# luisdamiano/sparseRGPs

Hardware: AMD Instinct MI355X
Metric: sparse-GP objective+gradient evals/sec at n=1e6, m=1024, d=8 (higher is better)
Workload: dtype f64; 1 GPU; C3: Titsias VI ELBO + gradient, n=1000000, m=1024, d=8, ard, P=10, knots fixed; n=1000000, m=1024, d=8, kernel=ard, parallelism=single

## Files before the change

### sparsergps_amd/_build.py

```python
from __future__ import annotations

import os
import shutil
import subprocess

HERE = os.path.dirname(os.path.abspath(__file__))
ROOT = os.path.dirname(HERE)
CSRC = os.path.join(HERE, "csrc")
LIBDIR = os.path.join(HERE, "lib")
LIB = os.path.join(LIBDIR, "libsgp.so")
VARIANT_ROOT = os.path.join(ROOT, "tools", "ab")
SOURCES = ["capi.hip", "k_cov.hip", "k_mfma.hip", "k_dense.hip", "k_lap.hip", "multi.hip"]
CSRC_HEADERS = ["sgp_internal.h", "sgp_probe.h", "sgp_multi.h", "sgp_pool.h", "sgp_syrk_plan.h"]
HEADERS = [*CSRC_HEADERS,
           os.path.join("..", "..", "include", "sgp.h"),
           os.path.join("..", "..", "include", "sgp_diag.h")]
ARCH = "gfx950"


class HipccMissing(RuntimeError):
    """No hipcc on this machine (the only case in which an existing library may be reused)."""


def hipcc():
    for cand in (shutil.which("hipcc"), "/opt/rocm/bin/hipcc"):
        if cand and os.path.exists(cand):
            return cand
    raise HipccMissing("hipcc not found: cannot build libsgp.so")


FILE_FLAGS = {"k_dense.hip": ["-mllvm", "-amdgpu-mfma-vgpr-form"]}


def _compile_flags(src, defs=()):
    return ["-O3", f"--offload-arch={ARCH}", "-std=c++17", "-fPIC", "-Wno-unused-result",
            *FILE_FLAGS.get(src, []), *defs]


def _compile_cmd(cc, src, obj, defs=(), csrc=CSRC):
    return [cc, *_compile_flags(src, defs), "-c", os.path.join(csrc, src), "-o", obj]


LINK_FLAGS = [f"--offload-arch={ARCH}", "-shared", "-fPIC", "-ldl", "-lpthread"]


def _link_cmd(cc, objs, out):
    return [cc, *LINK_FLAGS, "-o", out] + list(objs)


def _stamp(path):
    return path + ".cmd"


def _read_stamp(path):
    try:
        with open(_stamp(path)) as f:
            return f.read()
    except OSError:
        return None


def _write_stamp(path, key):
    with open(_stamp(path), "w") as f:
        f.write(key)


def _obj_key(src, defs):
    return "\0".join([src, *_compile_flags(src, defs)])


def _lib_key(objs):
    return "\0".join([*LINK_FLAGS, *(os.path.basename(o) for o in objs)])


def _obj_stale(obj, key, src, csrc=CSRC):
    if not os.path.exists(obj) or _read_stamp(obj) != key:
        return True
    t = os.path.getmtime(obj)
    deps = [os.path.join(csrc, src)] + [os.path.join(csrc, h) for h in HEADERS]
    return any(os.path.getmtime(p) > t for p in deps if os.path.exists(p))


def _sources(csrc=CSRC):
    return [s for s in SOURCES if csrc == CSRC or os.path.exists(os.path.join(csrc, s))]


def _plan(outdir, defs, csrc=CSRC):
    objs, todo = [], []
    for src in _sources(csrc):
        obj = os.path.join(outdir, src.replace(".hip", ".o"))
        objs.append(obj)
        if _obj_stale(obj, _obj_key(src, defs), src, csrc):
            todo.append((src, obj))
    return objs, todo


def _lib_stale(lib, objs):
    if not os.path.exists(lib) or _read_stamp(lib) != _lib_key(objs):
        return True
    t = os.path.getmtime(lib)
    return any(os.path.getmtime(o) > t for o in objs)


def _build_into(outdir, lib, defs, force, verbose, csrc=CSRC):
    cc = hipcc()
    os.makedirs(outdir, exist_ok=True)
    objs, todo = _plan(outdir, defs, csrc)
    if force:
        todo = list(zip(_sources(csrc), objs))
    procs = []
    for src, obj in todo:
        cmd = _compile_cmd(cc, src, obj, defs, csrc)
        procs.append((src, cmd, obj,
                      subprocess.Popen(cmd, stdout=subprocess.PIPE, stderr=subprocess.STDOUT)))
    failed = None
    for src, cmd, obj, p in procs:
        out, _ = p.communicate()
        if p.returncode != 0:
            failed = failed or f"hipcc failed ({' '.join(cmd)}):\n{out.decode(errors='replace')}"
            continue
        _write_stamp(obj, _obj_key(src, defs))
        if verbose and out:
            print(out.decode(errors="replace"))
    if failed:
        raise RuntimeError(failed)
    if not force and not todo and not _lib_stale(lib, objs):
        return lib
    tmp = lib + ".tmp"
    res = subprocess.run(_link_cmd(cc, objs, tmp), stdout=subprocess.PIPE, stderr=subprocess.STDOUT)
    if res.returncode != 0:
        raise RuntimeError(f"link failed:\n{res.stdout.decode(errors='replace')}")
    os.replace(tmp, lib)
    _write_stamp(lib, _lib_key(objs))
    return lib


def stale() -> bool:
    objs, todo = _plan(LIBDIR, ())
    return bool(todo) or _lib_stale(LIB, objs)


def build(force: bool = False, verbose: bool = False) -> str:
    if os.environ.get("SGP_HIPCC_DEFS"):
        raise RuntimeError("SGP_HIPCC_DEFS is not honoured by the product build; "
                           "use sparsergps_amd._build.build_variant() for A/B libraries")
    return _build_into(LIBDIR, LIB, (), force, verbose)


def build_variant(name: str, defs=(), force: bool = False, verbose: bool = False,
                  rev: str | None = None) -> str:
    if not name or "/" in name or name.startswith("."):
        raise ValueError(f"bad variant name {name!r}")
    defs = ["-DSGP_PROBE_BUILD", *defs]
    outdir = os.path.join(VARIANT_ROOT, name)
    csrc = CSRC
    if rev is not None:
        src_root = os.path.join(outdir, "src")
        os.makedirs(src_root, exist_ok=True)
        for path in ["sparsergps_amd/csrc/" + f for f in SOURCES + CSRC_HEADERS] + ["include/sgp.h", "include/sgp_diag.h"]:
            res = subprocess.run(["git", "-C", ROOT, "show", f"{rev}:{path}"],
                                 stdout=subprocess.PIPE, stderr=subprocess.PIPE)
            if res.returncode != 0:
                continue
            out = res.stdout
            dst = os.path.join(src_root, path)
            os.makedirs(os.path.dirname(dst), exist_ok=True)
            old = open(dst, "rb").read() if os.path.exists(dst) else None
            if old != out:
                with open(dst, "wb") as f:
                    f.write(out)
        csrc = os.path.join(src_root, "sparsergps_amd", "csrc")
    return _build_into(outdir, os.path.join(outdir, "libsgp.so"), defs, force, verbose, csrc)


if __name__ == "__main__":
    import sys
    if len(sys.argv) > 2 and sys.argv[1] == "variant":
        rest = sys.argv[3:]
        rev = rest.pop(0) if rest and not rest[0].startswith("-") else None
        print(build_variant(sys.argv[2], rest, verbose=True, rev=rev))
    else:
        print(build(force=True, verbose=True))
```

### sparsergps_amd/csrc/k_mfma.hip

```cpp
#include <algorithm>
#include <vector>

#include "sgp_internal.h"
#include "sgp_probe.h"
#include "sgp_syrk_plan.h"

namespace {

constexpr int T128 = 128;
constexpr int BK = 16;
constexpr int SB = 144;
constexpr int SA = 17;
constexpr int SYRK_RGRP = 16;

__device__ __forceinline__ double wave_sum(double v) {
#pragma unroll
  for (int o = 32; o > 0; o >>= 1) v += __shfl_xor(v, o, 64);
  return v;
}

__device__ __forceinline__ int64_t xcd_remap(int64_t orig, int64_t nwg) {
  return sgp_plan::xcd_remap(orig, nwg);
}

__device__ __forceinline__ void load8(const double* __restrict__ g, double2 (&v)[4]) {
  const double2* p = reinterpret_cast<const double2*>(g);
#pragma unroll
  for (int q = 0; q < 4; ++q) v[q] = p[q];
}
__device__ __forceinline__ void store8(double* s, const double2 (&v)[4]) {
  double2* p = reinterpret_cast<double2*>(s);
#pragma unroll
  for (int q = 0; q < 4; ++q) p[q] = v[q];
}

__device__ __forceinline__ void syrk_group(int64_t gi, int nb, int wv, int& ta, int& tb, int& rs,
                                           int& cs, int& rp, int& cp) {
  const int64_t noff = (int64_t)nb * (nb - 1) / 2;
  if (gi < noff) {
    int a = (int)((sqrtf(8.0f * (float)gi + 1.0f) + 1.0f) * 0.5f);
    while ((int64_t)a * (a - 1) / 2 > gi) --a;
    while ((int64_t)(a + 1) * a / 2 <= gi) ++a;
    const int b = (int)(gi - (int64_t)a * (a - 1) / 2);
    ta = a; tb = b;
    const int wr = wv >> 1, wc = wv & 1;
    rs = wr; cs = 2 + wc;
    rp = 2 * a + wr; cp = 2 * b + wc;
    return;
  }
  const int g = (int)(gi - noff), G = (3 * nb + 3) / 4;
  const int te = G + g / 3, kind = g % 3;
  ta = g;
  tb = (te < nb) ? te : g;
  if (wv == 0) { rs = 0; cs = 0; rp = 2 * g; cp = 2 * g; }
  else if (wv == 1) { rs = 1; cs = 0; rp = 2 * g + 1; cp = 2 * g; }
  else if (wv == 2) { rs = 1; cs = 1; rp = 2 * g + 1; cp = 2 * g + 1; }
  else if (te < nb) {
    if (kind == 0) { rs = 2; cs = 2; rp = 2 * te; cp = 2 * te; }
    else if (kind == 1) { rs = 3; cs = 2; rp = 2 * te + 1; cp = 2 * te; }
    else { rs = 3; cs = 3; rp = 2 * te + 1; cp = 2 * te + 1; }
  } else {
    rs = cs = rp = cp = -1;
  }
}

struct SyrkTMap {
  signed char e[128];
  int S;
};

template <bool SPREAD = false, int PAT = 0, int NVMEM = 8, int NMFMA = 64>
__device__ __forceinline__ void mfma_interleave() {
#pragma unroll
  for (int i = 0; i < NMFMA; ++i) {
    __builtin_amdgcn_sched_group_barrier(0x008, 1, 0);
    if (i >= SGP_IL_VMEM0 && i < SGP_IL_VMEM0 + NVMEM)
      __builtin_amdgcn_sched_group_barrier(0x020, 1, 0);
    if (SPREAD ? (i & 1) == 0 : i < 32)
      __builtin_amdgcn_sched_group_barrier(0x100, 1, 0);
    constexpr int w0 = PAT == 2 ? NMFMA - 8 : PAT == 3 ? NMFMA / 2 : NMFMA - 16;
    if (PAT != 4 && i >= w0 && i < w0 + 8)
      __builtin_amdgcn_sched_group_barrier(0x200, 1, 0);
  }
}

template <int V, int WMODE, int TMODE, bool COMPACT = false>
__device__ __forceinline__ void syrk_dt_body(const double* __restrict__ K, int64_t mp,
                                             const double* __restrict__ w,
                                             const double* __restrict__ r,
                                             const double* __restrict__ tv, int t, int64_t rbeg,
                                             int nsteps, double (*Ka)[BK * SB], double (*ws)[BK],
                                             double (*rw)[BK], double& tacc, double& rrp,
                                             double* __restrict__ out) {
  constexpr int R0 = V, R1 = 7 - V, N0 = R0 + 1, N1 = R1 + 1;
  constexpr bool WITH_T = TMODE != 0;
  const int tid = threadIdx.x, lane = tid & 63;
  d4 acc0[N0], acc1[N1];
#pragma unroll
  for (int c = 0; c < N0; ++c) acc0[c] = d4{0.0, 0.0, 0.0, 0.0};
#pragma unroll
  for (int c = 0; c < N1; ++c) acc1[c] = d4{0.0, 0.0, 0.0, 0.0};
  const int lrow = tid >> 4, lc = tid & 15;
  const double2* gA = reinterpret_cast<const double2*>(K + (rbeg + lrow) * mp + t * (int64_t)T128) + lc;
  const int64_t gstep = BK * mp / 2;
  double2 v[4];
  double vw = 1.0, vsa = 1.0, vrr = 0.0, vr = 0.0;
  double t4[4] = {0.0, 0.0, 0.0, 0.0};
  const int tcol = tid & (T128 - 1), trow = tid >> 7;
#define SDT_GLOAD(step)                                                         \
  {                                                                             \
    const int64_t o_ = (int64_t)(step) * gstep;                                 \
    const int64_t rr_ = rbeg + (int64_t)(step) * BK + (tid & (BK - 1));        \
    _Pragma("unroll") for (int q = 0; q < 4; ++q) v[q] = gA[o_ + 16 * q];       \
    if constexpr (WMODE == 1) vw = w[rr_];                                      \
    if constexpr (WMODE == 2) vsa = w[rbeg + (int64_t)(step) * BK + lrow];      \
    if constexpr (WITH_T) {                                                     \
      vrr = r[rr_];                                                             \
      if constexpr (TMODE == 2) vr = tv[rr_];                                   \
    }                                                                           \
  }
#define SDT_SSTORE(buf, fold)                                                   \
  {                                                                             \
    double2* p_ = reinterpret_cast<double2*>(&Ka[buf][lrow * SB]) + lc;         \
    _Pragma("unroll") for (int q = 0; q < 4; ++q) {                             \
      double2 x_ = v[q];                                                        \
      if constexpr (WMODE == 2) { x_.x *= vsa; x_.y *= vsa; }                   \
      p_[16 * q] = x_;                                                          \
    }                                                                           \
    if constexpr (WMODE == 1) ws[buf][tid & (BK - 1)] = vw;                     \
    if constexpr (WITH_T) {                                                     \
      const double rw_ = TMODE == 2 ? vr : vw * vrr;                            \
      rw[buf][tid & (BK - 1)] = rw_;                                            \
      rrp = fma(rw_ * (fold), vrr, rrp);                                        \
    }                                                                           \
  }
  if (nsteps > 0) {
    SDT_GLOAD(0);
    SDT_SSTORE(0, 1.0);
  }
  __syncthreads();
  for (int step = 0; step < nsteps; ++step) {
    const int cur = step & 1;
    const bool more = step + 1 < nsteps;
    SDT_GLOAD(more ? step + 1 : step);
    const double* Kc = Ka[cur];
#pragma unroll
    for (int kk = 0; kk < 4; ++kk) {
      const int krow = kk * 4 + (lane >> 4);
      const double* row = Kc + krow * SB + (lane & 15);
      double a0 = row[R0 * 16], a1 = row[R1 * 16];
      if constexpr (WMODE == 1) {
        const double wk = ws[cur][krow];
        a0 *= wk;
        a1 *= wk;
      }
#pragma unroll
      for (int c = 0; c < N1; ++c) {
        const double b = row[c * 16];
        if (c < N0) acc0[c] = __builtin_amdgcn_mfma_f64_16x16x4f64(a0, b, acc0[c], 0, 0, 0);
        acc1[c] = __builtin_amdgcn_mfma_f64_16x16x4f64(a1, b, acc1[c], 0, 0, 0);
      }
    }
    if constexpr (WITH_T) {
#pragma unroll
      for (int k = 0; k < BK / 2; ++k) {
        const int q = trow + 2 * k;
        t4[k & 3] = fma(rw[cur][q], Kc[q * SB + tcol], t4[k & 3]);
      }
    }
    SDT_SSTORE(cur ^ 1, more ? 1.0 : 0.0);
    if constexpr (SGP_SDT_IL && WMODE != 1) mfma_interleave<false, 2, 4, 36>();
    __syncthreads();
  }
#undef SDT_GLOAD
#undef SDT_SSTORE
  tacc = (t4[0] + t4[1]) + (t4[2] + t4[3]);
#pragma unroll
  for (int c = 0; c < N1; ++c)
#pragma unroll
    for (int hh = 0; hh < 2; ++hh) {
      if (hh == 0 && c >= N0) continue;
      const int R = hh == 0 ? R0 : R1;
      const d4& a = hh == 0 ? acc0[c] : acc1[c];
      const int rp = 2 * t + R / 4, cp = 2 * t + c / 4;
      double* blk = out + (COMPACT ? (int64_t)(R / 4 + c / 4)
                                   : (int64_t)(rp * (rp + 1) / 2 + cp)) * 4096;
#pragma unroll
      for (int q = 0; q < 4; ++q)
        blk[((R % 4) * 16 + (lane >> 4) + 4 * q) * 64 + (c % 4) * 16 + (lane & 15)] = a[q];
    }
}

template <int WMODE, int TMODE>
__device__ __forceinline__ void syrk_dtile(const double* __restrict__ K, int64_t n_pad,
                                           int64_t mp, const double* __restrict__ w,
                                           const double* __restrict__ r,
                                           const double* __restrict__ tv, int t, int nb,
                                           int64_t sd, int64_t chunk, double (*Ka)[BK * SB],
                                           double (*ws)[BK], double (*rw)[BK],
                                           double* __restrict__ out,
                                           double* __restrict__ slab_t,
                                           double* __restrict__ slab_rr) {
  const int64_t rbeg = sd * chunk;
  int64_t rend = rbeg + chunk;
  if (rend > n_pad) rend = n_pad;
  const int nsteps = rend > rbeg ? (int)((rend - rbeg) / BK) : 0;
  double tacc = 0.0, rrp = 0.0;
  switch (threadIdx.x >> 6) {
    case 0: syrk_dt_body<0, WMODE, TMODE>(K, mp, w, r, tv, t, rbeg, nsteps, Ka, ws, rw, tacc, rrp, out); break;
    case 1: syrk_dt_body<1, WMODE, TMODE>(K, mp, w, r, tv, t, rbeg, nsteps, Ka, ws, rw, tacc, rrp, out); break;
    case 2: syrk_dt_body<2, WMODE, TMODE>(K, mp, w, r, tv, t, rbeg, nsteps, Ka, ws, rw, tacc, rrp, out); break;
    default: syrk_dt_body<3, WMODE, TMODE>(K, mp, w, r, tv, t, rbeg, nsteps, Ka, ws, rw, tacc, rrp, out); break;
  }
  if constexpr (TMODE != 0) {
    const int tid = threadIdx.x;
    double* tsh = &Ka[0][0];
    tsh[tid] = tacc;
    __syncthreads();
    if (tid < T128) slab_t[(sd * nb + t) * T128 + tid] = tsh[tid] + tsh[tid + T128];
    if (t == 0 && tid < 64) {
      double v = tid < BK ? rrp : 0.0;
#pragma unroll
      for (int o = 32; o > 0; o >>= 1) v += __shfl_xor(v, o, 64);
      if (tid == 0) slab_rr[sd] = v;
    }
  }
}

template <int TMODE, int WMODE, int TR = 2>
__global__ void __launch_bounds__(256, 2)
k_syrk_blk(const double* __restrict__ K, int64_t n_pad, int64_t mp, const double* __restrict__ w,
           const double* __restrict__ r, const double* __restrict__ tv,
           int64_t chunk, int ngroups, int nb, double* __restrict__ slab,
           double* __restrict__ slab_t, double* __restrict__ slab_rr, SyrkTMap tm,
           int64_t nwg_blk, int64_t chunk_d, double* __restrict__ slab_d) {
  __shared__ __attribute__((aligned(16))) double Ka[2][BK * SB];
  __shared__ __attribute__((aligned(16))) double Kb[2][BK * SB];
  __shared__ double ws[2][BK];
  __shared__ double rw[2][BK];

  if constexpr (TMODE == 0 || WMODE == 3) {
    if ((int64_t)blockIdx.x >= nwg_blk) {
      const int64_t loc = (int64_t)blockIdx.x - nwg_blk;
      const int t = (int)(loc % nb);
      const int64_t sd = loc / nb;
      syrk_dtile<WMODE == 3 ? 1 : WMODE, TMODE>(
          K, n_pad, mp, w, r, tv, t, nb, sd, chunk_d, Ka, ws, rw,
          slab_d + sd * ((int64_t)(2 * nb) * (2 * nb + 1) / 2) * 4096, slab_t, slab_rr);
      return;
    }
  }
  const int64_t nwg = nwg_blk;
  const int64_t wgid = xcd_remap(blockIdx.x, nwg);
  const int split = (int)(wgid / ngroups);
  const int64_t gi = wgid % ngroups;
  const int tid = threadIdx.x, lane = tid & 63, wv = tid >> 6;
  int ta, tb, rs, cs, rp, cp;
  syrk_group(gi, nb, wv, ta, tb, rs, cs, rp, cp);
  const bool active = rs >= 0;
  const int64_t noff = (int64_t)nb * (nb - 1) / 2;
  const int dg = (gi >= noff) ? (int)(gi - noff) : -1;
  constexpr bool WITH_T = TMODE != 0 && WMODE != 3;
  constexpr bool with_t = WITH_T;
  static_assert(!(WMODE == 2 && TMODE != 0), "sqrt(w)-scaled images: S only");
  constexpr bool SCALE_A = WMODE == 2 || WMODE == 3, SCALE_B = WMODE == 2;
  int tmap = -1;
  if (with_t) {
    if (tm.S > 0) tmap = (int)tm.e[gi];
    else if (gi < noff) tmap = (tb == 0) ? ta : -1;
    else if (dg == 0) tmap = 0;
  }
  const int tS = (with_t && tm.S > 0) ? tm.S : 1, tW = T128 / tS;
  const int tpan = tmap >= 0 ? tmap / tS : -1;
  const int tng = 256 / tW, trg = tid / tW;
  const int tcol = tmap >= 0 ? (tmap % tS) * tW + tid % tW : 0;
  const bool t_on = with_t && tmap >= 0;
  const bool t_inb = tpan != ta;
  const bool t_rr = with_t && dg == 0 && tid < BK;
  double rrp = 0.0;
  double tacc4[4] = {0.0, 0.0, 0.0, 0.0}, vrr = 0.0, vr = 0.0;
  const int64_t rbeg = (int64_t)split * chunk;
  int64_t rend = rbeg + chunk;
  if (rend > n_pad) rend = n_pad;
  const int nsteps = (int)((rend - rbeg) / BK);

  d4 acc[4][4];
#pragma unroll
  for (int a = 0; a < 4; ++a)
#pragma unroll
    for (int b = 0; b < 4; ++b) acc[a][b] = d4{0.0, 0.0, 0.0, 0.0};

  const int lrow = tid >> 4, lc = tid & 15;
  constexpr bool has_tv = TMODE == 2;
  const double2* gA = reinterpret_cast<const double2*>(K + (rbeg + lrow) * mp + ta * (int64_t)T128) + lc;
  const double2* gB = reinterpret_cast<const double2*>(K + (rbeg + lrow) * mp + tb * (int64_t)T128) + lc;
  const int64_t gstep = BK * mp / 2;
  double2 va0, va1, va2, va3, vb0, vb1, vb2, vb3;
  double vw = 1.0, vsa = 1.0;
  const int ra = (rs >> 1) & 1, ro = (rs & 1) * 64;
  const int ca_ = (cs >> 1) & 1, co = (cs & 1) * 64;

#define SYRKB_GLOAD(step)                                                       \
  {                                                                             \
    const int64_t o_ = (int64_t)(step) * gstep;                                 \
    va0 = gA[o_]; va1 = gA[o_ + 16]; va2 = gA[o_ + 32]; va3 = gA[o_ + 48];      \
    vb0 = gB[o_]; vb1 = gB[o_ + 16]; vb2 = gB[o_ + 32]; vb3 = gB[o_ + 48];      \
              \
    const int64_t rr_ = rbeg + (int64_t)(step) * BK + (tid & (BK - 1));        \
    if constexpr (WMODE == 1) vw = w[rr_];                                      \
    if constexpr (SCALE_A) vsa = w[rbeg + (int64_t)(step) * BK + lrow];        \
    if constexpr (WITH_T) {                                                     \
      vrr = r[rr_];                                                             \
      if constexpr (has_tv) vr = tv[rr_];                                       \
    }                                                                           \
  }
#define SYRKB_SSTORE(buf, fold)                                                 \
  {                                                                             \
    double2* pa_ = reinterpret_cast<double2*>(&Ka[buf][lrow * SB]) + lc;        \
    double2* pb_ = reinterpret_cast<double2*>(&Kb[buf][lrow * SB]) + lc;        \
    if constexpr (SCALE_A) {              \
      va0.x *= vsa; va0.y *= vsa; va1.x *= vsa; va1.y *= vsa;                   \
      va2.x *= vsa; va2.y *= vsa; va3.x *= vsa; va3.y *= vsa;                   \
    }                                                                           \
    if constexpr (SCALE_B) {                                                    \
      vb0.x *= vsa; vb0.y *= vsa; vb1.x *= vsa; vb1.y *= vsa;                   \
      vb2.x *= vsa; vb2.y *= vsa; vb3.x *= vsa; vb3.y *= vsa;                   \
    }                                                                           \
    pa_[0] = va0; pa_[16] = va1; pa_[32] = va2; pa_[48] = va3;                  \
    pb_[0] = vb0; pb_[16] = vb1; pb_[32] = vb2; pb_[48] = vb3;                  \
    if constexpr (WMODE == 1) ws[buf][tid & (BK - 1)] = vw;                     \
    if constexpr (WITH_T) {                                                     \
      double rw_;                                          \
      if constexpr (has_tv) rw_ = vr;                                           \
      else rw_ = vw * vrr;                                                      \
      rw[buf][tid & (BK - 1)] = rw_;                                            \
      rrp = fma(rw_ * (fold), vrr, rrp);       \
// ... 388 lines not shown
  d4 acc0[N0], acc1[N1];
#pragma unroll
  for (int c = 0; c < N0; ++c) acc0[c] = d4{0.0, 0.0, 0.0, 0.0};
#pragma unroll
  for (int c = 0; c < N1; ++c) acc1[c] = d4{0.0, 0.0, 0.0, 0.0};
  const int lrow = tid >> 4, lc = tid & 15;
  const double2* gK = reinterpret_cast<const double2*>(K + (rbeg + lrow) * 256) + lc;
  constexpr int64_t gstep = BK * 256 / 2;
  double2 v[8];
  double vw = 1.0;
#define S256_GLOAD(step)                                                        \
  {                                                                             \
    const int64_t o_ = (int64_t)(step) * gstep;                                 \
    _Pragma("unroll") for (int q = 0; q < 8; ++q) v[q] = gK[o_ + 16 * q];       \
    if constexpr (WEIGHTED) vw = w[rbeg + (int64_t)(step) * BK + (tid & (BK - 1))]; \
  }
#define S256_SSTORE(buf)                                                        \
  {                                                                             \
    double2* p_ = reinterpret_cast<double2*>(&Ks[buf][lrow * SB2]) + lc;        \
    _Pragma("unroll") for (int q = 0; q < 8; ++q) p_[16 * q] = v[q];            \
    if constexpr (WEIGHTED) ws[buf][tid & (BK - 1)] = vw;                       \
  }
  if (nsteps > 0) {
    S256_GLOAD(0);
    S256_SSTORE(0);
  }
  __syncthreads();
  for (int step = 0; step < nsteps; ++step) {
    const int cur = step & 1;
    S256_GLOAD(step + 1 < nsteps ? step + 1 : step);
    const double* Kc = Ks[cur];
#pragma unroll
    for (int kk = 0; kk < 4; ++kk) {
      const int krow = kk * 4 + (lane >> 4);
      const double* row = Kc + krow * SB2 + (lane & 15);
      double a0 = row[R0 * 16], a1 = row[R1 * 16];
      if constexpr (WEIGHTED) {
        const double wk = ws[cur][krow];
        a0 *= wk;
        a1 *= wk;
      }
#pragma unroll
      for (int c = 0; c < N1; ++c) {
        const double b = row[c * 16];
        if (c < N0) acc0[c] = __builtin_amdgcn_mfma_f64_16x16x4f64(a0, b, acc0[c], 0, 0, 0);
        acc1[c] = __builtin_amdgcn_mfma_f64_16x16x4f64(a1, b, acc1[c], 0, 0, 0);
      }
    }
    S256_SSTORE(cur ^ 1);
    if constexpr (SGP_S256_IL) mfma_interleave<false, 2, 8, 68>();
    __syncthreads();
  }
#undef S256_GLOAD
#undef S256_SSTORE
#pragma unroll
  for (int c = 0; c < N1; ++c)
#pragma unroll
    for (int hh = 0; hh < 2; ++hh) {
      if (hh == 0 && c >= N0) continue;
      const int R = hh == 0 ? R0 : R1;
      const d4& a = hh == 0 ? acc0[c] : acc1[c];
      const int rp = R / 4, cp = c / 4;
      double* blk = out + (int64_t)(rp * (rp + 1) / 2 + cp) * 4096;
#pragma unroll
      for (int q = 0; q < 4; ++q)
        blk[((R % 4) * 16 + (lane >> 4) + 4 * q) * 64 + (c % 4) * 16 + (lane & 15)] = a[q];
    }
}

template <bool WEIGHTED>
__global__ void __launch_bounds__(256, 2)
k_syrk_s256(const double* __restrict__ K, int64_t n_pad, const double* __restrict__ w,
            int64_t chunk, double* __restrict__ slab) {
  __shared__ __attribute__((aligned(16))) double Ks[2][BK * SB2];
  __shared__ double ws[2][BK];
  const int64_t nwg = (int64_t)gridDim.x;
  const int64_t wgid = xcd_remap(blockIdx.x, nwg);
  const int64_t split = wgid >> 1;
  const int v = (int)(wgid & 1) * 4 + (threadIdx.x >> 6);
  const int64_t rbeg = split * chunk;
  int64_t rend = rbeg + chunk;
  if (rend > n_pad) rend = n_pad;
  const int nsteps = rend > rbeg ? (int)((rend - rbeg) / BK) : 0;
  double* out = slab + split * 10 * 4096;
#define S256_CASE(v_)                                                          \
  case v_:                                                                     \
    syrk256_body<v_, WEIGHTED>(K, w, rbeg, nsteps, Ks, ws, out);               \
    break;
  switch (v) {
    S256_CASE(0) S256_CASE(1) S256_CASE(2) S256_CASE(3)
    S256_CASE(4) S256_CASE(5) S256_CASE(6) S256_CASE(7)
  }
#undef S256_CASE
}

__global__ void __launch_bounds__(256, 2)
k_gemm_tn(const double* __restrict__ A, int64_t lda, const double* __restrict__ B, int64_t ldb,
          int64_t n_pad, int nta, int ntb, int64_t chunk, double* __restrict__ slab) {
  __shared__ __attribute__((aligned(16))) double Ka[2][BK * SB];
  __shared__ __attribute__((aligned(16))) double Kb[2][BK * SB];
  const int64_t nwg = (int64_t)gridDim.x;
  const int64_t wgid = xcd_remap(blockIdx.x, nwg);
  const int ntile = nta * ntb;
  const int split = (int)(wgid / ntile);
  const int tile = (int)(wgid % ntile);
  const int ta = tile / ntb, tb = tile % ntb;
  const int tid = threadIdx.x, lane = tid & 63, wv = tid >> 6;
  const int wr = wv >> 1, wc = wv & 1;
  const int64_t rbeg = (int64_t)split * chunk;
  int64_t rend = rbeg + chunk;
  if (rend > n_pad) rend = n_pad;
  const int nsteps = (int)((rend - rbeg) / BK);
  d4 acc[4][4];
#pragma unroll
  for (int a = 0; a < 4; ++a)
#pragma unroll
    for (int b = 0; b < 4; ++b) acc[a][b] = d4{0.0, 0.0, 0.0, 0.0};
  const int lrow = tid >> 4, lc = tid & 15;
  const double2* gA = reinterpret_cast<const double2*>(A + (rbeg + lrow) * lda + ta * (int64_t)T128) + lc;
  const double2* gB = reinterpret_cast<const double2*>(B + (rbeg + lrow) * ldb + tb * (int64_t)T128) + lc;
  const int64_t sa = BK * lda / 2, sb = BK * ldb / 2;
  double2 va0, va1, va2, va3, vb0, vb1, vb2, vb3;
#define TN_GLOAD(step)                                                          \
  {                                                                             \
    const int64_t oa_ = (int64_t)(step) * sa, ob_ = (int64_t)(step) * sb;       \
    va0 = gA[oa_]; va1 = gA[oa_ + 16]; va2 = gA[oa_ + 32]; va3 = gA[oa_ + 48];  \
    vb0 = gB[ob_]; vb1 = gB[ob_ + 16]; vb2 = gB[ob_ + 32]; vb3 = gB[ob_ + 48];  \
  }
#define TN_SSTORE(buf)                                                          \
  {                                                                             \
    double2* pa_ = reinterpret_cast<double2*>(&Ka[buf][lrow * SB]) + lc;        \
    double2* pb_ = reinterpret_cast<double2*>(&Kb[buf][lrow * SB]) + lc;        \
    pa_[0] = va0; pa_[16] = va1; pa_[32] = va2; pa_[48] = va3;                  \
    pb_[0] = vb0; pb_[16] = vb1; pb_[32] = vb2; pb_[48] = vb3;                  \
  }
  if (nsteps > 0) {
    TN_GLOAD(0);
    TN_SSTORE(0);
  }
  __syncthreads();
  for (int step = 0; step < nsteps; ++step) {
    const int cur = step & 1;
    if (step + 1 < nsteps) TN_GLOAD(step + 1);
    const double* As = Ka[cur];
    const double* Bs = Kb[cur];
#pragma unroll
    for (int kk = 0; kk < 4; ++kk) {
      const int krow = kk * 4 + (lane >> 4);
      double af[4], bf[4];
#pragma unroll
      for (int f = 0; f < 4; ++f) {
        af[f] = As[krow * SB + wr * 64 + f * 16 + (lane & 15)];
        bf[f] = Bs[krow * SB + wc * 64 + f * 16 + (lane & 15)];
      }
#pragma unroll
      for (int fm = 0; fm < 4; ++fm)
#pragma unroll
        for (int fn = 0; fn < 4; ++fn)
          acc[fm][fn] = __builtin_amdgcn_mfma_f64_16x16x4f64(af[fm], bf[fn], acc[fm][fn], 0, 0, 0);
    }
    if (step + 1 < nsteps) TN_SSTORE(cur ^ 1);
    __syncthreads();
  }
#undef TN_GLOAD
#undef TN_SSTORE
  double* out = slab + ((int64_t)split * ntile + tile) * (T128 * T128);
#pragma unroll
  for (int fm = 0; fm < 4; ++fm)
#pragma unroll
    for (int fn = 0; fn < 4; ++fn)
#pragma unroll
      for (int q = 0; q < 4; ++q) {
        const int row = wr * 64 + fm * 16 + (lane >> 4) + 4 * q;
        const int col = wc * 64 + fn * 16 + (lane & 15);
        out[row * T128 + col] = acc[fm][fn][q];
      }
}

__global__ void __launch_bounds__(256)
k_gemm_tn_reduce(const double* __restrict__ slab, int splits, int nta, int ntb,
                 double* __restrict__ C) {
  const int tile = blockIdx.y;
  const int e = blockIdx.x * 256 + threadIdx.x;
  const int ntile = nta * ntb;
  double s = 0.0;
  for (int sp = 0; sp < splits; ++sp) s += slab[((int64_t)sp * ntile + tile) * (T128 * T128) + e];
  const int ta = tile / ntb, tb = tile % ntb;
  const int64_t a = (int64_t)ta * T128 + e / T128, b = (int64_t)tb * T128 + e % T128;
  C[a * (int64_t)ntb * T128 + b] = s;
}

__global__ void __launch_bounds__(256)
k_syrk_reduce_t(const double* __restrict__ slab_t, const double* __restrict__ slab_rr,
                int splits, int nb, int64_t mp, double* __restrict__ red) {
  const int64_t a = (int64_t)blockIdx.x * 256 + threadIdx.x;
  if (a < mp) {
    const int ta = (int)(a / T128), col = (int)(a % T128);
    double s = 0.0;
    for (int sp = 0; sp < splits; ++sp) s += slab_t[((int64_t)sp * nb + ta) * T128 + col];
    red[mp * mp + a] = s;
  }
  if (blockIdx.x == 0 && threadIdx.x == 0) {
    double s = 0.0;
    for (int sp = 0; sp < splits; ++sp) s += slab_rr[sp];
    red[mp * mp + mp] = s;
  }
}

enum { EPI_GRAD = 0, EPI_ROWQUAD = 1 };

constexpr int CON_A_SZ = T128 * SA;
constexpr int CON_B_SZ = BK * SB;
constexpr int CON_LDS = 2 * (CON_A_SZ + CON_B_SZ);

enum { CON_FULL = 0, CON_TAIL = 1, CON_HEAD = 2 };
constexpr int64_t CON_SK_SLOT = 65 * 256;
struct ConSK {
  double* ws = nullptr;
  int dp = -1;
  unsigned* flags = nullptr;
  unsigned epoch = 0;
  int64_t slot = 0;
  int* status = nullptr;
};

__device__ __forceinline__ unsigned con_ldu_sc1(const unsigned* p) {
  return __hip_atomic_load(p, __ATOMIC_RELAXED, __HIP_MEMORY_SCOPE_AGENT);
}

template <int DT, int EPI, bool V2, bool KNOT, bool FROM_T, bool KU, bool T2, int SKM,
          bool VIF = false>
__device__ __forceinline__ void con_tile(
    const KernParams& kp, const double* __restrict__ K, const double* __restrict__ M,
    const double* __restrict__ X, int64_t ldx, int64_t n, int64_t n_pad,
    const double* __restrict__ U, int64_t ldu, int64_t m, int64_t mp, const ConArgs& ca,
    double* __restrict__ slab, int nrec, double* __restrict__ rowq, int64_t ti, int64_t tj,
    int64_t wgid, int kb, int ke, double* lds, double (*red)[SGP_MAXD + 5], double (*s_uk)[BK],
    const ConSK& sk, int part, int tid_in) {
  const double* __restrict__ r = ca.r;
  const double* __restrict__ uvec = ca.uvec;
  const double* __restrict__ cdiag = ca.cdiag;
  constexpr int A_SZ = CON_A_SZ, B_SZ = CON_B_SZ;
  const int64_t ntj = mp / T128;
  const int64_t nwg = (n_pad / T128) * ntj;
  const int64_t i0 = ti * T128, j0 = tj * T128;

  const int tid = tid_in, lane = tid & 63, wv = tid >> 6;
  const int wr = wv >> 1, wc = wv & 1;
  const bool with_u = KU && (uvec != nullptr) && (ca.alpha_in == nullptr);
  constexpr bool with_v = V2;
  constexpr bool NOCS = VIF && !KNOT;

  d4 acc[4][4];
#pragma unroll
  for (int a = 0; a < 4; ++a)
#pragma unroll
    for (int b = 0; b < 4; ++b) acc[a][b] = d4{0.0, 0.0, 0.0, 0.0};

  const int arow = tid >> 1, acol = (tid & 1) * 8;
  const double2* gA = reinterpret_cast<const double2*>(K + (i0 + arow) * mp + acol);
  const int bk = tid >> 4, bc = tid & 15;
  const double2* gB = reinterpret_cast<const double2*>(M + (int64_t)bk * mp + j0) + bc;
  const int64_t bstep = BK * mp / 2;
  double2 va0, va1, va2, va3, vb0, vb1, vb2, vb3;
  double ku = 0.0, vuk = 0.0;
  const double* __restrict__ uk_src = with_u ? uvec : M;

#define CON_GLOAD(step)                                                          \
  {                                                                              \
    const int64_t oa_ = (int64_t)(step) * (BK / 2), ob_ = (int64_t)(step) * bstep; \
    va0 = gA[oa_]; va1 = gA[oa_ + 1]; va2 = gA[oa_ + 2]; va3 = gA[oa_ + 3];      \
    vb0 = gB[ob_]; vb1 = gB[ob_ + 16]; vb2 = gB[ob_ + 32]; vb3 = gB[ob_ + 48];   \
    if constexpr (KU) vuk = uk_src[(int64_t)(step) * BK + (tid & (BK - 1))];     \
  }
#define CON_SSTORE(buf)                                                          \
  {                                                                              \
    double* As_ = lds + (buf) * (A_SZ + B_SZ);                                   \
    double* pa_ = &As_[arow * SA + acol];                                        \
    double2* pb_ = reinterpret_cast<double2*>(&As_[A_SZ + bk * SB]) + bc;        \
    pa_[0] = va0.x; pa_[1] = va0.y; pa_[2] = va1.x; pa_[3] = va1.y;              \
    pa_[4] = va2.x; pa_[5] = va2.y; pa_[6] = va3.x; pa_[7] = va3.y;              \
    pb_[0] = vb0; pb_[16] = vb1; pb_[32] = vb2; pb_[48] = vb3;                   \
    if constexpr (KU) s_uk[buf][tid & (BK - 1)] = vuk;    \
  }
#define CON_KU(buf)                                                              \
  {                                                                              \
    const double* u_ = &s_uk[buf][acol];                                         \
    ku = fma(va0.x, u_[0], ku); ku = fma(va0.y, u_[1], ku);                      \
    ku = fma(va1.x, u_[2], ku); ku = fma(va1.y, u_[3], ku);                      \
    ku = fma(va2.x, u_[4], ku); ku = fma(va2.y, u_[5], ku);                      \
    ku = fma(va3.x, u_[6], ku); ku = fma(va3.y, u_[7], ku);                      \
  }

  SGP_PROBE_CON_STAMP(0);
  if constexpr (FROM_T) {
#pragma unroll
    for (int fm = 0; fm < 4; ++fm)
#pragma unroll
      for (int fn = 0; fn < 4; ++fn)
#pragma unroll
        for (int q = 0; q < 4; ++q)
          acc[fm][fn][q] = ca.tin[(i0 + wr * 64 + fm * 16 + (lane >> 4) + 4 * q) * mp + j0 +
                                  wc * 64 + fn * 16 + (lane & 15)];
  } else {
  CON_GLOAD(kb);
  CON_SSTORE(0);
  __syncthreads();
  for (int step = kb; step < ke; ++step) {
    const int cur = (step - kb) & 1;
    if constexpr (KU) CON_KU(cur);
    CON_GLOAD(step + 1 < ke ? step + 1 : step);
    const double* As = lds + cur * (A_SZ + B_SZ);
    const double* Bs = As + A_SZ;
#pragma unroll
    for (int kk = 0; kk < 4; ++kk) {
      const int kx = kk * 4 + (lane >> 4);
      double af[4], bf[4];
#pragma unroll
      for (int f = 0; f < 4; ++f) {
        af[f] = As[(wr * 64 + f * 16 + (lane & 15)) * SA + kx];
        bf[f] = Bs[kx * SB + wc * 64 + f * 16 + (lane & 15)];
      }
#pragma unroll
      for (int fm = 0; fm < 4; ++fm)
#pragma unroll
        for (int fn = 0; fn < 4; ++fn)
          acc[fm][fn] = __builtin_amdgcn_mfma_f64_16x16x4f64(af[fm], bf[fn], acc[fm][fn], 0, 0, 0);
    }
    CON_SSTORE(cur ^ 1);
    mfma_interleave<SGP_CON_IL_SPREAD, SGP_CON_IL_PAT>();
    __syncthreads();
  }
  }
#undef CON_GLOAD
#undef CON_SSTORE
#undef CON_KU

  if constexpr (SKM == CON_TAIL) {
    double* w = sk.ws + sk.slot * CON_SK_SLOT;
#pragma unroll
    for (int fm = 0; fm < 4; ++fm)
#pragma unroll
      for (int fn = 0; fn < 4; ++fn)
#pragma unroll
        for (int q = 0; q < 4; ++q)
          __hip_atomic_store(&w[((fm * 4 + fn) * 4 + q) * 256 + tid], acc[fm][fn][q],
                             __ATOMIC_RELAXED, __HIP_MEMORY_SCOPE_AGENT);
    __hip_atomic_store(&w[64 * 256 + tid], ku, __ATOMIC_RELAXED, __HIP_MEMORY_SCOPE_AGENT);
    asm volatile("s_waitcnt vmcnt(0)" ::: "memory");
    __syncthreads();
    if (tid == 0)
      __hip_atomic_store(&sk.flags[sk.slot], sk.epoch, __ATOMIC_RELAXED, __HIP_MEMORY_SCOPE_AGENT);
    return;
  }
  if (SKM == CON_HEAD && part == CON_HEAD) {
    if (tid == 0) {
      unsigned it = 0;
      while (con_ldu_sc1(&sk.flags[sk.slot]) != sk.epoch) {
        if (++it >= (1u << 22)) {
          atomicExch(sk.status, -1);
          break;
        }
        __builtin_amdgcn_s_sleep(1);
      }
    }
    __syncthreads();
    const double* w = sk.ws + sk.slot * CON_SK_SLOT;
#pragma unroll
    for (int fm = 0; fm < 4; ++fm) {
      double t[4][4];
#pragma unroll
      for (int fn = 0; fn < 4; ++fn)
#pragma unroll
        for (int q = 0; q < 4; ++q)
          t[fn][q] = __hip_atomic_load(&w[((fm * 4 + fn) * 4 + q) * 256 + tid], __ATOMIC_RELAXED,
                                       __HIP_MEMORY_SCOPE_AGENT);
#pragma unroll
      for (int fn = 0; fn < 4; ++fn)
#pragma unroll
        for (int q = 0; q < 4; ++q) acc[fm][fn][q] += t[fn][q];
      __builtin_amdgcn_sched_barrier(0);
    }
    ku += __hip_atomic_load(&w[64 * 256 + tid], __ATOMIC_RELAXED, __HIP_MEMORY_SCOPE_AGENT);
  }

  SGP_PROBE_CON_STAMP(1);
  if constexpr (SGP_CON_EPI_PRIO > 0) __builtin_amdgcn_s_setprio(SGP_CON_EPI_PRIO);
  SGP_PROBE_CON_SKIP_EPILOGUE()
  double* s_alpha = lds;
  double* s_rs = s_alpha + T128;
  double* s_u = s_rs + T128;
  double* s_cd = s_u + T128;
  double* s_beta = s_cd + T128;
  double* s_v = s_beta + T128;
  double* s_xs = s_v + T128;
  double* s_us = s_xs + T128 * 16;
  double* s_rs2 = lds + 8320;
  static_assert(8320 + T128 <= 2 * (A_SZ + B_SZ), "s_rs2 fits the LDS image");
  ku += __shfl_xor(ku, 1, 64);
  double a2 = 0.0;
  if ((tid & 1) == 0) {
    const int64_t i = i0 + arow;
    double iz, al;
    if constexpr (VIF) {
      iz = ca.invz;
      al = r[i] * iz;
    } else {
      iz = ca.invz_vec ? ca.invz_vec[i] : ca.invz;
      al = ca.alpha_in ? ca.alpha_in[i]
                       : (with_u ? (r[i] - ku) * iz : 0.0);
    }
    const bool iv = i < n;
    s_alpha[arow] = iv ? al : 0.0;
    s_rs[arow] = iv ? (ca.rs_vec ? ca.rs * ca.rs_vec[i] : ca.rs) : 0.0;
    if constexpr (T2) s_rs2[arow] = iv ? (ca.rs_vec2 ? ca.rs2 * ca.rs_vec2[i] : ca.rs2) : 0.0;
    s_beta[arow] = (with_v && iv) ? ca.beta_in[i] : 0.0;
    if constexpr (!VIF) {
      if (tj == 0) {
        if (ca.count_a2 && i < n) a2 = al * al;
        if (ca.alpha_out) ca.alpha_out[i] = al;
      }
    }
  }
  const double* Kt = K + i0 * mp + j0;

  if constexpr (EPI == EPI_ROWQUAD) {
    if (ca.tstore != nullptr) {
#pragma unroll
      for (int fm = 0; fm < 4; ++fm)
#pragma unroll
        for (int fn = 0; fn < 4; ++fn)
#pragma unroll
          for (int q = 0; q < 4; ++q)
            ca.tstore[(i0 + wr * 64 + fm * 16 + (lane >> 4) + 4 * q) * mp + j0 + wc * 64 +
                      fn * 16 + (lane & 15)] = acc[fm][fn][q];
    }
    __syncthreads();
    double* s_q = s_cd;
#pragma unroll
    for (int fm = 0; fm < 4; ++fm) {
      double kv[4][4];
#pragma unroll
      for (int q = 0; q < 4; ++q)
#pragma unroll
        for (int fn = 0; fn < 4; ++fn)
          kv[q][fn] = Kt[(int64_t)(wr * 64 + fm * 16 + (lane >> 4) + 4 * q) * mp +
                         wc * 64 + fn * 16 + (lane & 15)];
#pragma unroll
      for (int q = 0; q < 4; ++q) {
        const int row = wr * 64 + fm * 16 + (lane >> 4) + 4 * q;
        double v = 0.0;
#pragma unroll
        for (int fn = 0; fn < 4; ++fn)
          v = fma(kv[q][fn], acc[fm][fn][q], v);
        v += __shfl_xor(v, 1, 64);
        v += __shfl_xor(v, 2, 64);
        v += __shfl_xor(v, 4, 64);
        v += __shfl_xor(v, 8, 64);
        if ((lane & 15) == 0) s_q[wc * T128 + row] = v;
      }
    }
    __syncthreads();
    if (tid < T128) rowq[tj * n_pad + i0 + tid] = s_q[tid] + s_q[T128 + tid];
    return;
  } else {
    const int d = kp.d;
    constexpr int sus = 9;
    const bool ard = (kp.kernel == 1);
    const double rl2s = kp.rl2[0];
    const int L = kp.L;
    for (int e = tid; e < T128; e += 256) {
      const int64_t j = j0 + e;
      s_u[e] = (uvec && j < m) ? uvec[j] : 0.0;
      s_v[e] = (with_v && j < m) ? ca.vvec[j] : 0.0;
      s_cd[e] = (cdiag && j < m) ? cdiag[j] : 0.0;
    }
    double e_sig = 0.0;
    double e_sq = 0.0;
    double* s_kn;
    static_assert(DT % 8 == 0, "coordinates are processed in chunks of 8");
    constexpr int NCH = DT / 8;
    {
      constexpr int KST = 136;
      const double* const kq0 = K + (i0 + (wv >> 1) * 64 + 4 * (wv & 1)) * mp + j0 + 2 * lane;
      double* kst = s_us + ((T128 * sus + 1) & ~1);
#define CON_XSTAGE(ch_)                                                                  \
      _Pragma("unroll") for (int e = tid; e < T128 * 8; e += 256) {                      \
        const int rr = e % T128, c = e / T128, cg = 8 * (ch_) + c;                       \
        const int64_t i = i0 + rr, j = j0 + rr;                                          \
        double xv = 0.0;                                                                 \
        if (cg < d) {                                                                    \
          const double sc = ard ? kp.rl[cg] : 1.0;                                       \
          xv = (i < n) ? X[i + cg * ldx] * sc : 0.0;                                     \
          s_us[rr * sus + c] = (j < m) ? U[j + cg * ldu] * sc : 0.0;                     \
        }                                                                                \
        s_xs[rr * 16 + c] = xv;                                                          \
        s_xs[rr * 16 + 8 + c] = xv * xv;                                                 \
      }
#ifdef SGP_CON_PROBE_NO_KDMA
#define CON_KHALF(s_)
#else
#define CON_KHALF(s_)                                                                    \
      _Pragma("unroll") for (int q_ = 0; q_ < 4; ++q_) {                                 \
        const int rho_ = wv * 4 + q_;                                                    \
        __builtin_amdgcn_global_load_lds(                                                \
            (const __attribute__((address_space(1))) void*)(                             \
                kq0 + (int64_t)(((s_) >> 1) * 16 + ((s_) & 1) * 8 + q_) * mp),          \
            (__attribute__((address_space(3))) void*)(kst + ((s_) & 1) * 16 * KST + rho_ * KST), \
            16, 0, 0);                                                                   \
      }
#endif
      double t2n[2][4];
#define CON_T2LOAD(s_)                                                                   \
      if constexpr (T2) {                                                                \
        _Pragma("unroll") for (int r2_ = 0; r2_ < 2; ++r2_)                              \
        _Pragma("unroll") for (int fn_ = 0; fn_ < 4; ++fn_)                              \
          t2n[r2_][fn_] = ca.tin2[(i0 + wr * 64 + ((s_) >> 1) * 16 + (lane >> 4) +        \
                                   4 * (2 * ((s_) & 1) + r2_)) * mp + j0 + wc * 64 +      \
                                  fn_ * 16 + (lane & 15)];                                \
      }
      CON_KHALF(0);
      CON_KHALF(1);
      CON_T2LOAD(0);
      CON_XSTAGE(0);
      __builtin_amdgcn_s_waitcnt(0);
      __syncthreads();
      s_kn = kst;
      SGP_PROBE_CON_STAMP(4);

      d4 P[4];
      double Cc[4], ucol[4], vcol[4];
#pragma unroll
      for (int fn = 0; fn < 4; ++fn) {
        const int col = wc * 64 + fn * 16 + (lane & 15);
        P[fn] = d4{0.0, 0.0, 0.0, 0.0};
        Cc[fn] = 0.0;
        ucol[fn] = s_u[col];
        vcol[fn] = with_v ? s_v[col] : 0.0;
      }
      {
#pragma unroll
        for (int hs = 0; hs < 8; ++hs) {
          const int fm = hs >> 1, h = hs & 1;
          if (hs > 0) {
            __builtin_amdgcn_s_waitcnt(0);
            __syncthreads();
            if (hs < 7) { CON_KHALF(hs + 1); }
          }
          double t2c[2][4];
          if constexpr (T2) {
#pragma unroll
            for (int r2 = 0; r2 < 2; ++r2)
#pragma unroll
              for (int fn = 0; fn < 4; ++fn) t2c[r2][fn] = t2n[r2][fn];
            if (hs < 7) { CON_T2LOAD(hs + 1); }
          }
          const double* kb = kst + h * 16 * KST;
          double xb[2];
#pragma unroll
          for (int r2 = 0; r2 < 2; ++r2)
            xb[r2] = s_xs[(wr * 64 + fm * 16 + 4 * (2 * h + r2) + (lane >> 4)) * 16 + (lane & 15)];
#pragma unroll
          for (int fn = 0; fn < 4; ++fn) {
            const int col = wc * 64 + fn * 16 + (lane & 15);
            double kv[2];
#pragma unroll
            for (int r2 = 0; r2 < 2; ++r2) kv[r2] = kb[(wr * 8 + (lane >> 4) + 4 * r2) * KST + col];
#pragma unroll
            for (int r2 = 0; r2 < 2; ++r2) {
              const int q = 2 * h + r2;
              const int row = wr * 64 + fm * 16 + (lane >> 4) + 4 * q;
              double G = s_rs[row] * acc[fm][fn][q];
              if constexpr (T2) G = fma(s_rs2[row], t2c[r2][fn], G);
              if constexpr (V2) G = fma(s_beta[row], vcol[fn], G);
              G = fma(s_alpha[row], ucol[fn], G);
              double w = G * kv[r2];
              if constexpr ((V2 && KNOT) || FROM_T) w = (j0 + col < m && i0 + row < n) ? w : 0.0;
              if constexpr (!NOCS) Cc[fn] += w;
              acc[fm][fn][q] = w;
            }
          }
#pragma unroll
          for (int r2 = 0; r2 < 2; ++r2)
#pragma unroll
            for (int fn = 0; fn < 4; ++fn)
#ifndef SGP_CON_PROBE_NO_EPI_MFMA
              P[fn] = __builtin_amdgcn_mfma_f64_16x16x4f64(acc[fm][fn][2 * h + r2], xb[r2], P[fn],
                                                           0, 0, 0);
#else
              P[fn][r2] = fma(acc[fm][fn][2 * h + r2], xb[r2], P[fn][r2]);
#endif
          if (hs == 1) SGP_PROBE_CON_STAMP(3);
        }
        __syncthreads();
      }
#undef CON_KHALF
#undef CON_T2LOAD
      SGP_PROBE_CON_STAMP(5);
      const int cp = lane & 15, cc = cp & 7;
#pragma unroll
      for (int ch = 0; ch < NCH; ++ch) {
        if (8 * ch >= d) break;
        if (ch > 0) {
          __syncthreads();
          CON_XSTAGE(ch);
          __syncthreads();
// ... 1035 lines not shown
```

### sparsergps_amd/csrc/sgp_probe.h

```cpp
#pragma once

#if (defined(SGP_CON_TRACE) || defined(SGP_CON_NO_EPILOGUE) || defined(SGP_GJ_TRACE) ||       \
     defined(SGP_IL_VMEM0) || defined(SGP_CON_IL_PAT) || defined(SGP_SYRK_IL_PAT) ||          \
     defined(SGP_CON_IL_SPREAD) || defined(SGP_CON_SHMEM) ||                                  \
     defined(SGP_SYRK_BAL) || defined(SGP_SYRK_WB) || defined(SGP_SYRK_WB_SLOTS) ||           \
     defined(SGP_SDT_IL) || defined(SGP_S256_IL) ||                  \
     defined(SGP_SDT_W) || defined(SGP_SDT_WW) || defined(SGP_SDT_WT) ||                      \
     defined(SGP_SYRK_W3) || defined(SGP_CON_ROWQ_KU) ||                                      \
     defined(SGP_LAP_RS_CFG) || defined(SGP_GJ_MM_UNROLL) || defined(SGP_VI_BUILD_NO_T) ||        \
     defined(SGP_GJ_STEPS) || defined(SGP_GJ_GMAX) || defined(SGP_CHAIN_US_STEP) ||         \
     defined(SGP_CHAIN_US_FIX) || defined(SGP_HOST_PROBE) || defined(SGP_BUILD_OCC_T2) ||      \
     defined(SGP_CON_EPI_PRIO) || defined(SGP_CON_PROBE_NO_EPI_MFMA) ||                       \
     defined(SGP_CON_PROBE_NO_KDMA)) &&      \
    !defined(SGP_PROBE_BUILD)
#error "timing probes and experiment knobs are for variant builds only (SGP_PROBE_BUILD)"
#endif

#ifndef SGP_CON_EPI_PRIO
#define SGP_CON_EPI_PRIO 0
#endif
#ifndef SGP_BUILD_OCC_T2
#define SGP_BUILD_OCC_T2 4
#endif
#ifndef SGP_IL_VMEM0
#define SGP_IL_VMEM0 0
#endif
#ifndef SGP_CON_IL_PAT
#define SGP_CON_IL_PAT 2
#endif
#ifndef SGP_SYRK_IL_PAT
#define SGP_SYRK_IL_PAT 0
#endif
#ifndef SGP_CON_IL_SPREAD
#define SGP_CON_IL_SPREAD false
#endif
#ifndef SGP_CON_SHMEM
#define SGP_CON_SHMEM 0
#endif
#ifndef SGP_SYRK_BAL
#define SGP_SYRK_BAL 1
#endif
#ifndef SGP_SYRK_WB
#define SGP_SYRK_WB 1
#endif
#ifndef SGP_SYRK_WB_SLOTS
#define SGP_SYRK_WB_SLOTS 512
#endif
#ifndef SGP_SDT_IL
#define SGP_SDT_IL 1
#endif
#ifndef SGP_SDT_W
#define SGP_SDT_W 38
#endif
#ifndef SGP_SDT_WW
#define SGP_SDT_WW 2
#endif
#ifndef SGP_SDT_WT
#define SGP_SDT_WT 6
#endif
#ifndef SGP_SYRK_W3
#define SGP_SYRK_W3 1
#endif
#ifndef SGP_CON_ROWQ_KU
#define SGP_CON_ROWQ_KU 0
#endif
#ifndef SGP_LAP_RS_CFG
#define SGP_LAP_RS_CFG 0
#endif
#ifndef SGP_GJ_MM_UNROLL
#define SGP_GJ_MM_UNROLL 16
#endif
#ifndef SGP_S256_IL
#define SGP_S256_IL 0
#endif
#ifndef SGP_GJ_STEPS
#define SGP_GJ_STEPS 0
#endif
#ifndef SGP_GJ_GMAX
#define SGP_GJ_GMAX 128
#endif
#ifndef SGP_CHAIN_US_STEP
#define SGP_CHAIN_US_STEP 60.0
#endif
#ifndef SGP_CHAIN_US_FIX
#define SGP_CHAIN_US_FIX 250.0
#endif
#ifndef SGP_VI_BUILD_NO_T
#define SGP_VI_BUILD_NO_T 0
#endif

#ifdef SGP_CON_TRACE
#define SGP_PROBE_CON_STAMP(k_)        \
  do {                                 \
    if (tid == 0) SGP_CON_TRACE(k_);   \
  } while (0)
#else
#define SGP_PROBE_CON_STAMP(k_) \
  do {                          \
  } while (0)
#endif

#ifdef SGP_CON_NO_EPILOGUE
#define SGP_PROBE_CON_SKIP_EPILOGUE()                                                   \
  if constexpr (EPI == EPI_GRAD) {                                                      \
    double v_ = 0.0;                                                                    \
    _Pragma("unroll") for (int fm_ = 0; fm_ < 4; ++fm_)                                 \
      _Pragma("unroll") for (int fn_ = 0; fn_ < 4; ++fn_)                               \
        v_ += acc[fm_][fn_][0] + acc[fm_][fn_][3];                                      \
    if (v_ == 1234.5) slab[tid] = v_;                                                   \
    return;                                                                             \
  }
#else
#define SGP_PROBE_CON_SKIP_EPILOGUE()
#endif

#ifdef SGP_GJ_TRACE
#define SGP_PROBE_GJ_DECL() const bool gj_tr_ = (i == k + 1) && (j == k + 1) && threadIdx.x == 0
#define SGP_PROBE_GJ_STAMP(p_)          \
  do {                                  \
    if (gj_tr_) SGP_GJ_TRACE(k, p_);    \
  } while (0)
#else
#define SGP_PROBE_GJ_DECL() \
  do {                      \
  } while (0)
#define SGP_PROBE_GJ_STAMP(p_) \
  do {                         \
  } while (0)
#endif
```

Before: 21.40 evals/s.

## Stage contraction k-loop tiles via global_load_lds DMA with swizzled double-buffered LDS

```diff
diff --git a/sparsergps_amd/_build.py b/sparsergps_amd/_build.py
--- a/sparsergps_amd/_build.py
+++ b/sparsergps_amd/_build.py
@@ -11,7 +11,8 @@
 LIB = os.path.join(LIBDIR, "libsgp.so")
 VARIANT_ROOT = os.path.join(ROOT, "tools", "ab")
 SOURCES = ["capi.hip", "k_cov.hip", "k_mfma.hip", "k_dense.hip", "k_lap.hip", "multi.hip"]
-CSRC_HEADERS = ["sgp_internal.h", "sgp_probe.h", "sgp_multi.h", "sgp_pool.h", "sgp_syrk_plan.h"]
+CSRC_HEADERS = ["sgp_internal.h", "sgp_probe.h", "sgp_multi.h", "sgp_pool.h", "sgp_syrk_plan.h",
+                "sgp_kstage.h"]
 HEADERS = [*CSRC_HEADERS,
            os.path.join("..", "..", "include", "sgp.h"),
            os.path.join("..", "..", "include", "sgp_diag.h")]
diff --git a/sparsergps_amd/csrc/k_mfma.hip b/sparsergps_amd/csrc/k_mfma.hip
--- a/sparsergps_amd/csrc/k_mfma.hip
+++ b/sparsergps_amd/csrc/k_mfma.hip
@@ -2,6 +2,7 @@
 #include <vector>
 
 #include "sgp_internal.h"
+#include "sgp_kstage.h"
 #include "sgp_probe.h"
 #include "sgp_syrk_plan.h"
 
@@ -32,6 +33,41 @@
   double2* p = reinterpret_cast<double2*>(s);
 #pragma unroll
   for (int q = 0; q < 4; ++q) p[q] = v[q];
+}
+
+namespace ks = sgp_kstage;
+static_assert(ks::kKStride == SB && ks::kBK == BK && ks::kTile == T128, "sgp_kstage.h's k image");
+
+__device__ __forceinline__ void kst_dma16(const void* gbase, unsigned voff, unsigned lds_dst) {
+  unsigned keep;
+  asm volatile(
+      "s_mov_b32 %0, m0\n\t"
+      "s_mov_b32 m0, %3\n\t"
+      "s_nop 0\n\t"
+      "global_load_lds_dwordx4 %1, %2\n\t"
+      "s_mov_b32 m0, %0"
+      : "=&s"(keep)
+      : "v"(voff), "s"(gbase), "s"(lds_dst)
+      : "memory");
+}
+__device__ __forceinline__ void kst_dma_wait() { asm volatile("s_waitcnt vmcnt(0)" ::: "memory"); }
+__device__ __forceinline__ void kst_step_end() {
+  __builtin_amdgcn_sched_barrier(0);
+  kst_dma_wait();
+  __syncthreads();
+}
+__device__ __forceinline__ unsigned kst_lds_addr(const double* p) {
+  return __builtin_amdgcn_readfirstlane(
+      (unsigned)(uintptr_t)(__attribute__((address_space(3))) const void*)p);
+}
+__device__ __forceinline__ const void* kst_uniform(const void* p) {
+  const uint64_t a = (uint64_t)(uintptr_t)p;
+  const uint32_t lo = __builtin_amdgcn_readfirstlane((uint32_t)a);
+  const uint32_t hi = __builtin_amdgcn_readfirstlane((uint32_t)(a >> 32));
+  return (const void*)(uintptr_t)(((uint64_t)hi << 32) | lo);
+}
+__device__ __forceinline__ double kst_ld(const double* img, int byte_off) {
+  return *reinterpret_cast<const double*>(reinterpret_cast<const char*>(img) + byte_off);
 }
 
 __device__ __forceinline__ void syrk_group(int64_t gi, int nb, int wv, int& ta, int& tb, int& rs,
@@ -1026,6 +1062,67 @@
         for (int q = 0; q < 4; ++q)
           acc[fm][fn][q] = ca.tin[(i0 + wr * 64 + fm * 16 + (lane >> 4) + 4 * q) * mp + j0 +
                                   wc * 64 + fn * 16 + (lane & 15)];
+  } else if constexpr (SGP_KLOOP_DMA && VIF && !KU) {
+    static_assert(ks::kRowImgDoubles <= A_SZ && ks::kKImgDoubles == B_SZ, "DMA images fit the stage");
+    const int wvs = __builtin_amdgcn_readfirstlane(wv);
+    const int64_t rowb = mp * 8;
+    unsigned voa[ks::kInstr];
+#pragma unroll
+    for (int i = 0; i < ks::kInstr; ++i)
+      voa[i] = (unsigned)((ks::row_dma_row(wvs, i, lane) - ks::row_dma_row(wvs, i, 0)) * rowb) +
+               (unsigned)(ks::row_dma_chunk(wvs, i, lane) * ks::kDmaBytes);
+    const unsigned vob = ks::k_dma_chunk(lane) * ks::kDmaBytes;
+    const char* gMs = static_cast<const char*>(kst_uniform(M + j0));
+    const int64_t stepb = BK * rowb;
+    const char* gKr[ks::kInstr];
+    int64_t ko[ks::kInstr];
+#pragma unroll
+    for (int i = 0; i < ks::kInstr; ++i) {
+      gKr[i] = static_cast<const char*>(kst_uniform(K + (i0 + ks::row_dma_row(wvs, i, 0)) * mp));
+      ko[i] = ks::k_dma_krow(wvs, i) * rowb;
+    }
+    const unsigned l0 = kst_lds_addr(lds);
+    constexpr unsigned BUFB = (A_SZ + B_SZ) * 8, BOFF = A_SZ * 8;
+#define CON_DMA2(h, step, buf)                                                              \
+    _Pragma("unroll") for (int q_ = 2 * (h); q_ < 2 * (h) + 2; ++q_) {                      \
+      const int i_ = q_ & 3;                                                                \
+      if (q_ < 4)                                                                           \
+        kst_dma16(gKr[i_] + (int64_t)(step) * (BK * 8),                                     \
+                  voa[i_], l0 + (unsigned)(buf) * BUFB + ks::row_dma_lds(wvs, i_));         \
+      else                                                                                  \
+        kst_dma16(gMs + (int64_t)(step) * stepb + ko[i_], vob,                              \
+                  l0 + (unsigned)(buf) * BUFB + BOFF + ks::k_dma_lds(wvs, i_));             \
+    }
+    CON_DMA2(0, kb, 0);
+    CON_DMA2(1, kb, 0);
+    CON_DMA2(2, kb, 0);
+    CON_DMA2(3, kb, 0);
+    kst_dma_wait();
+    __syncthreads();
+    for (int step = kb; step < ke; ++step) {
+      const int cur = (step - kb) & 1;
+      const int nxt = step + 1 < ke ? step + 1 : step;
+      const double* As = lds + cur * (A_SZ + B_SZ);
+      const double* Bs = As + A_SZ;
+#pragma unroll
+      for (int kk = 0; kk < 4; ++kk) {
+        double af[4], bf[4];
+#pragma unroll
+        for (int f = 0; f < 4; ++f) {
+          af[f] = kst_ld(As, ks::row_frag(wr, f, kk, lane));
+          bf[f] = kst_ld(Bs, ks::k_frag(wc * 64, f, kk, lane));
+        }
+        CON_DMA2(kk, nxt, cur ^ 1);
+#pragma unroll
+        for (int fm = 0; fm < 4; ++fm)
+#pragma unroll
+          for (int fn = 0; fn < 4; ++fn)
+            acc[fm][fn] = __builtin_amdgcn_mfma_f64_16x16x4f64(af[fm], bf[fn], acc[fm][fn], 0, 0, 0);
+      }
+      mfma_interleave<SGP_CON_IL_SPREAD, 4, 0>();
+      kst_step_end();
+    }
+#undef CON_DMA2
   } else {
   CON_GLOAD(kb);
   CON_SSTORE(0);
diff --git a/sparsergps_amd/csrc/sgp_kstage.h b/sparsergps_amd/csrc/sgp_kstage.h
--- /dev/null
+++ b/sparsergps_amd/csrc/sgp_kstage.h
@@ -0,0 +1,65 @@
+#pragma once
+
+#include <stdint.h>
+
+#if defined(__HIPCC__)
+#ifndef SGP_HD
+#define SGP_HD __host__ __device__ inline
+#endif
+#else
+#ifndef SGP_HD
+#define SGP_HD inline
+#endif
+#endif
+
+namespace sgp_kstage {
+
+constexpr int kBK = 16;
+constexpr int kTile = 128;
+constexpr int kWaves = 4;
+constexpr int kLanes = 64;
+constexpr int kInstr = 4;
+constexpr int kDmaBytes = 16;
+constexpr int kPiece = kLanes * kDmaBytes;
+
+constexpr int kRowBytes = kBK * 8;
+constexpr int kRowPad = 128;
+constexpr int kRowImgBytes = kTile * kRowBytes + (kTile / 16) * kRowPad;
+constexpr int kRowImgDoubles = kRowImgBytes / 8;
+
+SGP_HD int row_swz(int row) { return (row >> 1) & 7; }
+SGP_HD int row_base(int row) { return row * kRowBytes + (row >> 4) * kRowPad; }
+
+SGP_HD int row_dma_group(int wave, int i) { return wave * kInstr + i; }
+SGP_HD int row_dma_lds(int wave, int i) { return row_base(row_dma_group(wave, i) * 8); }
+SGP_HD int row_dma_row(int wave, int i, int lane) { return row_dma_group(wave, i) * 8 + (lane >> 3); }
+SGP_HD int row_dma_chunk(int wave, int i, int lane) {
+  return (lane & 7) ^ row_swz(row_dma_row(wave, i, lane));
+}
+SGP_HD int row_elem(int row, int k) {
+  return row_base(row) + (((k >> 1) ^ row_swz(row)) << 4) + ((k & 1) << 3);
+}
+SGP_HD int row_frag_row(int wr, int fm, int lane) { return wr * 64 + fm * 16 + (lane & 15); }
+SGP_HD int row_frag_k(int kk, int lane) { return kk * 4 + (lane >> 4); }
+SGP_HD int row_frag(int wr, int fm, int kk, int lane) {
+  return row_elem(row_frag_row(wr, fm, lane), row_frag_k(kk, lane));
+}
+
+constexpr int kKStride = 144;
+constexpr int kKStrideBytes = kKStride * 8;
+constexpr int kKImgDoubles = kBK * kKStride;
+constexpr int kKImgBytes = kKImgDoubles * 8;
+
+SGP_HD int k_dma_krow(int wave, int i) { return wave * kInstr + i; }
+SGP_HD int k_dma_lds(int wave, int i) { return k_dma_krow(wave, i) * kKStrideBytes; }
+SGP_HD int k_dma_chunk(int lane) { return lane; }
+SGP_HD int k_elem(int k, int col) { return k * kKStrideBytes + col * 8; }
+SGP_HD int k_frag_k(int kk, int lane) { return kk * 4 + (lane >> 4); }
+SGP_HD int k_frag_col(int c0, int f, int lane) { return c0 + f * 16 + (lane & 15); }
+SGP_HD int k_frag(int c0, int f, int kk, int lane) {
+  return k_elem(k_frag_k(kk, lane), k_frag_col(c0, f, lane));
+}
+
+SGP_HD int bank_pair(int byte_off) { return (byte_off >> 3) & 31; }
+
+}
diff --git a/sparsergps_amd/csrc/sgp_probe.h b/sparsergps_amd/csrc/sgp_probe.h
--- a/sparsergps_amd/csrc/sgp_probe.h
+++ b/sparsergps_amd/csrc/sgp_probe.h
@@ -4,7 +4,7 @@
      defined(SGP_IL_VMEM0) || defined(SGP_CON_IL_PAT) || defined(SGP_SYRK_IL_PAT) ||          \
      defined(SGP_CON_IL_SPREAD) || defined(SGP_CON_SHMEM) ||                                  \
      defined(SGP_SYRK_BAL) || defined(SGP_SYRK_WB) || defined(SGP_SYRK_WB_SLOTS) ||           \
-     defined(SGP_SDT_IL) || defined(SGP_S256_IL) ||                  \
+     defined(SGP_SDT_IL) || defined(SGP_S256_IL) || defined(SGP_KLOOP_DMA) ||                 \
      defined(SGP_SDT_W) || defined(SGP_SDT_WW) || defined(SGP_SDT_WT) ||                      \
      defined(SGP_SYRK_W3) || defined(SGP_CON_ROWQ_KU) ||                                      \
      defined(SGP_LAP_RS_CFG) || defined(SGP_GJ_MM_UNROLL) || defined(SGP_VI_BUILD_NO_T) ||        \
@@ -45,6 +45,9 @@
 #endif
 #ifndef SGP_SYRK_WB_SLOTS
 #define SGP_SYRK_WB_SLOTS 512
+#endif
+#ifndef SGP_KLOOP_DMA
+#define SGP_KLOOP_DMA 1
 #endif
 #ifndef SGP_SDT_IL
 #define SGP_SDT_IL 1
```

After: 21.53 evals/s, median of 6. Within noise of the previous version (+0.6%).
